# ixaxaar/lambda-cdm-raytracing

Measured on NVIDIA B200. Metric: pairwise_interactions_per_s, higher is better.
Workload: dtype f32

## Files before the change

lambda-cdm-raytracing_b200/csrc/capi.cu:

```cuda
#include <math.h>
#include <new>
#include <string.h>

#include "common.cuh"
#include "diag.cuh"
#include "direct.cuh"
#include "ics.cuh"
#include "leapfrog.cuh"
#include "pm.cuh"
#include "probe.cuh"
#include "shard.cuh"
#include "sort.cuh"
#include "tree.cuh"

using namespace b200;

static inline cudaStream_t pick_stream(b200_ctx*, void* stream) { return (cudaStream_t)stream; }

extern "C" {

const char* b200_error_string(int status) {
    switch (status) {
        case B200_OK: return "ok";
        case B200_ERR_INVALID: return "invalid argument";
        case B200_ERR_NO_DEVICE: return "no usable sm_100 CUDA device (there is no CPU fallback)";
        case B200_ERR_STATE: return "call out of order";
        case B200_ERR_NOMEM: return "device allocation failed";
        case B200_ERR_UNSUPPORTED: return "unsupported configuration";
        default: break;
    }
    if (status >= 1000 && status < 2000) return cudaGetErrorString((cudaError_t)(status - 1000));
    if (status >= 2000 && status < 3000) return shard_error_string(status - 2000);
    if (status >= 3000 && status < 4000) return "cuFFT error (status - 3000 is the cufftResult)";
    return "unknown b200grav status";
}

int b200_abi_version(void) { return B200GRAV_ABI_VERSION; }

int b200_ctx_create(int device, size_t max_particles, b200_ctx** out) {
    if (!out) return B200_ERR_INVALID;
    *out = nullptr;
    int count = 0;
    if (cudaGetDeviceCount(&count) != cudaSuccess || count == 0) {
        cudaGetLastError();
        return B200_ERR_NO_DEVICE;
    }
    if (device < 0 || device >= count) return B200_ERR_INVALID;
    cudaDeviceProp prop;
    B200_CUDA(cudaGetDeviceProperties(&prop, device));
    if (prop.major != 10) return B200_ERR_NO_DEVICE;
    B200_CUDA(cudaSetDevice(device));
    b200_ctx* ctx = new (std::nothrow) b200_ctx();
    if (!ctx) return B200_ERR_NOMEM;
    ctx->device = device;
    ctx->sm_count = prop.multiProcessorCount;
    cudaError_t ce = cudaStreamCreateWithFlags(&ctx->stream, cudaStreamNonBlocking);
    if (ce == cudaSuccess) ce = cudaEventCreate(&ctx->ev0);
    if (ce == cudaSuccess) ce = cudaEventCreate(&ctx->ev1);
    if (ce != cudaSuccess) { b200_ctx_destroy(ctx); return 1000 + (int)ce; }
    if (max_particles) {
        int s = ctx->src_tiles.reserve(direct_tiles_bytes(max_particles));
        if (s != B200_OK) { b200_ctx_destroy(ctx); return s; }
    }
    *out = ctx;
    return B200_OK;
}

int b200_ctx_destroy(b200_ctx* ctx) {
    if (!ctx) return B200_OK;
    cudaSetDevice(ctx->device);
    if (ctx->stream) cudaStreamSynchronize(ctx->stream);
    tree_destroy(ctx);
    shard_finalize(ctx);
    pm_destroy(ctx);
    ctx->src_tiles.release(); ctx->partials.release(); ctx->mass_flag.release(); ctx->zero_flag.release();
    ctx->energy_part.release(); ctx->energy_phi.release(); ctx->energy_out.release();
    ctx->ic_wk.release(); ctx->ic_tmp.release(); ctx->ic_psi.release(); ctx->ic_stats.release();
    ctx->h_pos3.release(); ctx->h_vel3.release(); ctx->h_mass.release(); ctx->h_posm4.release(); ctx->h_acc3.release();
    ctx->h_tree_posm4.release();
    ctx->probe.release(); ctx->sort_scratch.release();
    if (ctx->ev0) cudaEventDestroy(ctx->ev0);
    if (ctx->ev1) cudaEventDestroy(ctx->ev1);
    if (ctx->stream) cudaStreamDestroy(ctx->stream);
    delete ctx;
    return B200_OK;
}

int b200_ctx_device(const b200_ctx* ctx) { return ctx ? ctx->device : -1; }
int b200_ctx_sm_count(const b200_ctx* ctx) { return ctx ? ctx->sm_count : 0; }

void* b200_ctx_stream(const b200_ctx* ctx) { return ctx ? (void*)ctx->stream : nullptr; }

int b200_ctx_sync(b200_ctx* ctx, void* stream) {
    if (!ctx) return B200_ERR_INVALID;
    B200_CUDA(cudaStreamSynchronize(stream ? (cudaStream_t)stream : ctx->stream));
    return B200_OK;
}

int b200_direct_forces_dev(b200_ctx* ctx, const void* posm4, size_t n_sources, size_t i0,
                           size_t n_targets, float eps, float box, void* acc3, void* stream) {
    if (!ctx) return B200_ERR_INVALID;
    if (n_targets == 0) return B200_OK;
    if (!posm4 || !acc3 || i0 + n_targets > n_sources) return B200_ERR_INVALID;
    if (!(eps > 0.f) || box < 0.f) return B200_ERR_INVALID;
    B200_CUDA(cudaSetDevice(ctx->device));
    cudaStream_t st = pick_stream(ctx, stream);
    B200_TRY(ctx->src_tiles.reserve(direct_tiles_bytes(n_sources)));
    B200_TRY(ctx->mass_flag.reserve(sizeof(int)));
    B200_TRY(direct_pack_tiles(ctx, posm4, n_sources, ctx->src_tiles.as<float>(), ctx->mass_flag.as<int>(), st));
    DirectSources src;
    memset(&src, 0, sizeof src);
    src.n_parts = 1;
    src.tiles[0] = ctx->src_tiles.as<float>();
    src.total_tiles = src.tile_end[0] = (int)((n_sources + DIRECT_TILE_J - 1) / DIRECT_TILE_J);
    return direct_forces(ctx, src, (const float4*)posm4 + i0, n_targets, eps, box, acc3,
                         ctx->mass_flag.as<int>(), st);
}

int b200_direct_potential_dev(b200_ctx* ctx, const void* posm4, size_t n_sources, size_t i0,
                              size_t n_targets, float eps, float box, void* phi, void* stream) {
    if (!ctx) return B200_ERR_INVALID;
    if (n_targets == 0) return B200_OK;
    if (!posm4 || !phi || i0 + n_targets > n_sources) return B200_ERR_INVALID;
    if (!(eps > 0.f) || box < 0.f) return B200_ERR_INVALID;
    B200_CUDA(cudaSetDevice(ctx->device));
    cudaStream_t st = pick_stream(ctx, stream);
    B200_TRY(ctx->src_tiles.reserve(direct_tiles_bytes(n_sources)));
    B200_TRY(ctx->mass_flag.reserve(sizeof(int)));
    B200_TRY(direct_pack_tiles(ctx, posm4, n_sources, ctx->src_tiles.as<float>(), ctx->mass_flag.as<int>(), st));
    DirectSources src;
    memset(&src, 0, sizeof src);
    src.n_parts = 1;
    src.tiles[0] = ctx->src_tiles.as<float>();
    src.total_tiles = src.tile_end[0] = (int)((n_sources + DIRECT_TILE_J - 1) / DIRECT_TILE_J);
    return direct_potential(ctx, src, (const float4*)posm4 + i0, n_targets, eps, box, phi,
                            ctx->mass_flag.as<int>(), st);
}

int b200_energy_dev(b200_ctx* ctx, const void* posm4, size_t n_sources, size_t i0, size_t n_targets,
                    const void* vel3, float eps, float box, double* kinetic, double* potential,
                    void* stream) {
    if (!ctx || !kinetic || !potential) return B200_ERR_INVALID;
    *kinetic = *potential = 0.0;
    if (n_targets == 0) return B200_OK;
    if (!posm4 || !vel3 || i0 + n_targets > n_sources) return B200_ERR_INVALID;
    B200_CUDA(cudaSetDevice(ctx->device));
    cudaStream_t st = pick_stream(ctx, stream);
    B200_TRY(ctx->energy_phi.reserve(n_targets * sizeof(float)));
    B200_TRY(ctx->energy_out.reserve(2 * sizeof(double)));
    B200_TRY(b200_direct_potential_dev(ctx, posm4, n_sources, i0, n_targets, eps, box, ctx->energy_phi.p, stream));
    B200_TRY(energy_reduce(ctx, (const float4*)posm4 + i0, vel3, ctx->energy_phi.p, n_targets,
                           ctx->energy_out.as<double>(), st));
    double h[2];
    B200_CUDA(cudaMemcpyAsync(h, ctx->energy_out.p, sizeof h, cudaMemcpyDeviceToHost, st));
    B200_CUDA(cudaStreamSynchronize(st));
    *kinetic = h[0];
    *potential = h[1];
    return B200_OK;
}

int b200_force_error_dev(b200_ctx* ctx, const void* acc_test, const void* acc_ref, size_t n,
                         double* avg_rel_error, double* max_rel_error, void* stream) {
    if (!ctx || !avg_rel_error || !max_rel_error) return B200_ERR_INVALID;
    *avg_rel_error = *max_rel_error = 0.0;
    if (n == 0) return B200_OK;
    if (!acc_test || !acc_ref) return B200_ERR_INVALID;
    B200_CUDA(cudaSetDevice(ctx->device));
    return force_error(ctx, acc_test, acc_ref, n, avg_rel_error, max_rel_error, pick_stream(ctx, stream));
}
// ... 572 lines not shown
```

lambda-cdm-raytracing_b200/csrc/common.cuh:

```cuda
#pragma once
#ifdef B200_BOUNDS_CHECK
#include <assert.h>
#define B200_DEV_ASSERT(c) assert(c)
#else
#define B200_DEV_ASSERT(c) ((void)0)
#endif

#include <cuda_runtime.h>
#include <stddef.h>
#include <stdint.h>

#include "b200grav.h"

#define B200_CUDA(call)                                   \
    do {                                                  \
        cudaError_t e__ = (call);                         \
        if (e__ != cudaSuccess) return 1000 + (int)e__;   \
    } while (0)

#define B200_TRY(call)                  \
    do {                                \
        int s__ = (call);               \
        if (s__ != B200_OK) return s__; \
    } while (0)

struct DevBuf {
    void* p = nullptr;
    size_t bytes = 0;
    int reserve(size_t need) {
        if (need <= bytes) return B200_OK;
        if (p) cudaFree(p);
        p = nullptr; bytes = 0;
        size_t want = need + need / 8 + 256;
        cudaError_t e = cudaMalloc(&p, want);
        if (e != cudaSuccess) { cudaGetLastError(); return B200_ERR_NOMEM; }
        bytes = want;
        return B200_OK;
    }
    void release() { if (p) cudaFree(p); p = nullptr; bytes = 0; }
    template <class T> T* as() const { return (T*)p; }
};

namespace b200 { struct TreeState; struct ShardState; struct PmState; }

constexpr int B200_MAX_KERNEL_CFG = 64;
struct KernelCfg { const void* fn; int blocks_per_sm; };

struct b200_ctx {
    int device = 0;
    int sm_count = 0;
    cudaStream_t stream = nullptr;
    cudaEvent_t ev0 = nullptr, ev1 = nullptr;
    bool timing = false;
    float last_ms = 0.f;
    uint64_t launches = 0;
    KernelCfg kernel_cfg[B200_MAX_KERNEL_CFG];
    int n_kernel_cfg = 0;

    DevBuf src_tiles;
    DevBuf partials;
    DevBuf zero_flag;
    DevBuf mass_flag;
    DevBuf energy_part, energy_phi, energy_out;
    DevBuf ic_wk, ic_tmp, ic_psi, ic_stats;
    DevBuf h_pos3, h_vel3, h_mass, h_posm4, h_acc3;
    DevBuf h_tree_posm4;
    DevBuf probe, sort_scratch;

    b200::TreeState* tree = nullptr;
    b200::ShardState* shard = nullptr;
    b200::PmState* pm = nullptr;
};

static inline int ceil_div_i(long long a, long long b) { return (int)((a + b - 1) / b); }
```

lambda-cdm-raytracing_b200/csrc/direct.cu:

```cuda
#include <stdio.h>
#include <stdlib.h>

#include "common.cuh"
#include "direct.cuh"

namespace b200 {

namespace {

typedef unsigned long long u64;

__device__ __forceinline__ u64 pk(float lo, float hi) {
    u64 r;
    asm("mov.b64 %0, {%1, %2};" : "=l"(r) : "f"(lo), "f"(hi));
    return r;
}
__device__ __forceinline__ void unpk(u64 v, float& lo, float& hi) {
    asm("mov.b64 {%0, %1}, %2;" : "=f"(lo), "=f"(hi) : "l"(v));
}
__device__ __forceinline__ u64 add2(u64 a, u64 b) {
    u64 r;
    asm("add.rn.f32x2 %0, %1, %2;" : "=l"(r) : "l"(a), "l"(b));
    return r;
}
__device__ __forceinline__ u64 mul2(u64 a, u64 b) {
    u64 r;
    asm("mul.rn.f32x2 %0, %1, %2;" : "=l"(r) : "l"(a), "l"(b));
    return r;
}
__device__ __forceinline__ u64 fma2(u64 a, u64 b, u64 c) {
    u64 r;
    asm("fma.rn.f32x2 %0, %1, %2, %3;" : "=l"(r) : "l"(a), "l"(b), "l"(c));
    return r;
}
__device__ __forceinline__ float rsqrt_approx(float x) {
    float r;
    asm("rsqrt.approx.ftz.f32 %0, %1;" : "=f"(r) : "f"(x));
    return r;
}

__device__ __forceinline__ uint32_t smem_u32(const void* p) {
    return (uint32_t)__cvta_generic_to_shared(p);
}
__device__ __forceinline__ void mbar_init(uint64_t* bar, uint32_t count) {
    asm volatile("mbarrier.init.shared::cta.b64 [%0], %1;" ::"r"(smem_u32(bar)), "r"(count));
}
__device__ __forceinline__ void mbar_expect_tx(uint64_t* bar, uint32_t bytes) {
    asm volatile("mbarrier.arrive.expect_tx.shared::cta.b64 _, [%0], %1;" ::"r"(smem_u32(bar)),
                 "r"(bytes)
                 : "memory");
}
__device__ __forceinline__ void mbar_wait(uint64_t* bar, uint32_t parity) {
    asm volatile(
        "{\n"
        ".reg .pred p;\n"
        "WAIT_LOOP:\n"
        "mbarrier.try_wait.parity.shared::cta.b64 p, [%0], %1;\n"
        "@p bra WAIT_DONE;\n"
        "bra WAIT_LOOP;\n"
        "WAIT_DONE:\n"
        "}\n" ::"r"(smem_u32(bar)),
        "r"(parity)
        : "memory");
}
__device__ __forceinline__ void tma_load_1d(void* dst_smem, const void* src_gmem, uint32_t bytes,
                                            uint64_t* bar) {
    asm volatile(
        "cp.async.bulk.shared::cluster.global.mbarrier::complete_tx::bytes [%0], [%1], %2, [%3];" ::"r"(
            smem_u32(dst_smem)),
        "l"(src_gmem), "r"(bytes), "r"(smem_u32(bar))
        : "memory");
}

constexpr float FAR_AWAY = 1.0e18f;

__global__ void pack_tiles_kernel(const float4* __restrict__ posm, long long n, long long n_padded,
                                  float* __restrict__ tiles, int* __restrict__ mass_diff) {
    long long j = (long long)blockIdx.x * blockDim.x + threadIdx.x;
    if (j >= n_padded) return;
    float4 p = make_float4(FAR_AWAY, FAR_AWAY, FAR_AWAY, 0.f);
    if (j < n) {
        p = posm[j];
        if (mass_diff && p.w != posm[0].w) atomicAdd(mass_diff, 1);
    }
    long long t = j / DIRECT_TILE_J;
    int o = (int)(j % DIRECT_TILE_J);
    float* base = tiles + t * (4 * DIRECT_TILE_J) + o;
    base[0 * DIRECT_TILE_J] = p.x;
    base[1 * DIRECT_TILE_J] = p.y;
    base[2 * DIRECT_TILE_J] = p.z;
    base[3 * DIRECT_TILE_J] = p.w;
}

constexpr int STAGES = 4;
constexpr int TILE_J = DIRECT_TILE_J;
constexpr int TILE_FLOATS = 4 * TILE_J;
constexpr uint32_t TILE_BYTES = TILE_FLOATS * sizeof(float);

__device__ __forceinline__ const float* tile_ptr(const DirectSources& src, int t) {
    int p = 0, base = 0;
#pragma unroll 1
    while (p < src.n_parts - 1 && t >= src.tile_end[p]) { base = src.tile_end[p]; ++p; }
    return src.tiles[p] + (size_t)(t - base) * TILE_FLOATS;
}

constexpr int PMODE_OPEN = 0, PMODE_FLOAT = 1, PMODE_FIXED_XY = 2;

__device__ __forceinline__ uint32_t fixed_point(float x, double units_per_length) {
    uint32_t e = (uint32_t)(unsigned long long)__double2ll_rn((double)x * units_per_length);
    return e - (e >> 31);
}

__device__ __forceinline__ int sub3(uint32_t a, uint32_t b, uint32_t c) {
    int d;
    asm("vsub.s32.s32.s32.add %0, %1, %2, %3;" : "=r"(d) : "r"(a), "r"(b), "r"(c));
    return d;
}

template <int R, int THREADS, int MINB, int PMODE, bool UNIT, bool POT = false>
__global__ void __launch_bounds__(THREADS, MINB)
direct_kernel(const DirectSources src, const float4* __restrict__ targets, long long n_targets,
              float eps2, float box, double* __restrict__ partials, long long n_units, int n_tiles,
              const int* __restrict__ mass_diff) {
    constexpr bool PERIODIC = (PMODE == PMODE_FLOAT);
    constexpr bool FIXED = (PMODE == PMODE_FIXED_XY);
    static_assert(!(FIXED && POT), "the potential keeps the FP32 minimum image");
    if (mass_diff != nullptr) {
        const bool uniform = (*mass_diff == 0);
        if (uniform != UNIT) return;
    } else if (UNIT) {
        return;
    }
    constexpr int BLOCK_I = THREADS * R;
    extern __shared__ __align__(128) unsigned char smem_raw[];
    float* stage_buf = reinterpret_cast<float*>(smem_raw);
    uint64_t* full = reinterpret_cast<uint64_t*>(smem_raw + STAGES * TILE_BYTES);
    double* dsum = reinterpret_cast<double*>(smem_raw + STAGES * TILE_BYTES + 64);

    const int tid = threadIdx.x;
    const long long G = gridDim.x, c = blockIdx.x;
    const long long u0 = (c * n_units) / G, u1 = ((c + 1) * n_units) / G;
    if (u0 >= u1) return;
    const long long my_units = u1 - u0;

    if (tid == 0) {
#pragma unroll
        for (int s = 0; s < STAGES; ++s) mbar_init(&full[s], 1);
        asm volatile("fence.mbarrier_init.release.cluster;" ::: "memory");
    }
    __syncthreads();

    long long b = u0 / n_tiles;
    int t = (int)(u0 % n_tiles);

    if (tid == 0) {
        int tt = t;
        for (int k = 0; k < STAGES - 1 && k < my_units; ++k) {
            mbar_expect_tx(&full[k], TILE_BYTES);
            tma_load_1d(stage_buf + k * TILE_FLOATS, tile_ptr(src, tt), TILE_BYTES, &full[k]);
            if (++tt == n_tiles) tt = 0;
        }
    }
    int t_issue = (int)((u0 + (STAGES - 1)) % n_tiles);

    [[maybe_unused]] const double units = FIXED ? 4294967296.0 / (double)box : 1.0;
    [[maybe_unused]] const uint32_t zero = (uint32_t)(n_tiles >> 31);
    const u64 eps2_2 = pk(eps2, eps2);
    constexpr int RF = FIXED ? 1 : R, RI = FIXED ? R : 1;
    [[maybe_unused]] u64 nxi[RF], nyi[RF];
    u64 nzi[R];
    [[maybe_unused]] uint32_t ixi[RI], iyi[RI];
    auto load_targets = [&](long long blk) {
#pragma unroll
        for (int r = 0; r < R; ++r) {
            long long i = blk * BLOCK_I + r * THREADS + tid;
            float4 p = make_float4(0.f, 0.f, 0.f, 0.f);
            if (i < n_targets) p = targets[i];
            if constexpr (FIXED) {
                if (!(p.x == p.x) || !(p.y == p.y)) p.z = p.x + p.y;
                ixi[r] = fixed_point(p.x, units);
                iyi[r] = fixed_point(p.y, units);
            } else {
                nxi[r] = pk(-p.x, -p.x);
                nyi[r] = pk(-p.y, -p.y);
            }
// ... 91 lines not shown
                if constexpr (UNIT) f = mul2(f, rinv);
                else f = mul2(f, mul2(M, rinv));
                ax[r] = fma2(f, dx, ax[r]);
                ay[r] = fma2(f, dy, ay[r]);
                az[r] = fma2(f, dz, az[r]);
            }
        };

#pragma unroll 1
        for (int j4 = 0; j4 < TILE_J / 4; ++j4) {
            const ulonglong2 X = sx[j4], Y = sy[j4], Z = sz[j4];
            ulonglong2 M = make_ulonglong2(0ull, 0ull);
            if constexpr (!UNIT || FIXED) M = sm[j4];
            interact(X.x, Y.x, Z.x, M.x);
            interact(X.y, Y.y, Z.y, M.y);
        }

#pragma unroll
        for (int r = 0; r < R; ++r) {
            float lo, hi;
            unpk(ax[r], lo, hi); dsum[(0 * R + r) * THREADS + tid] += (double)(lo + hi);
            if constexpr (!POT) {
                unpk(ay[r], lo, hi); dsum[(1 * R + r) * THREADS + tid] += (double)(lo + hi);
                unpk(az[r], lo, hi); dsum[(2 * R + r) * THREADS + tid] += (double)(lo + hi);
            }
        }
        if constexpr (FIXED) asm volatile("fence.proxy.async.shared::cta;" ::: "memory");
        __syncthreads();

        ++t;
        const bool last = (k == my_units - 1);
        if (t == n_tiles || last) {
            double* rec = partials + (size_t)(c + b) * 3 * BLOCK_I;
#pragma unroll
            for (int r = 0; r < R; ++r) {
                rec[0 * BLOCK_I + r * THREADS + tid] = dsum[(0 * R + r) * THREADS + tid];
                if constexpr (!POT) {
                    rec[1 * BLOCK_I + r * THREADS + tid] = dsum[(1 * R + r) * THREADS + tid];
                    rec[2 * BLOCK_I + r * THREADS + tid] = dsum[(2 * R + r) * THREADS + tid];
                }
            }
            if (t == n_tiles) {
                t = 0;
                ++b;
                if (!last) load_targets(b);
            }
        }
    }
}

__global__ void direct_finalize_kernel(const double* __restrict__ partials, float* __restrict__ acc3,
                                       long long n_targets, int block_i, long long n_units,
                                       int n_tiles, int G, const int* __restrict__ mass_diff,
                                       const float* __restrict__ first_tile, double scale_xy) {
    long long i = (long long)blockIdx.x * blockDim.x + threadIdx.x;
    if (i >= n_targets) return;
    long long b = i / block_i;
    int o = (int)(i % block_i);
    long long uf = b * n_tiles, ul = uf + n_tiles - 1;
    long long cf = ((uf + 1) * G - 1) / n_units;
    long long cl = ((ul + 1) * G - 1) / n_units;
    double sx = 0.0, sy = 0.0, sz = 0.0;
    for (long long c = cf; c <= cl; ++c) {
        const double* rec = partials + (size_t)(c + b) * 3 * block_i;
        sx += rec[o];
        sy += rec[block_i + o];
        sz += rec[2 * block_i + o];
    }
    if (mass_diff != nullptr && *mass_diff == 0) {
        const double m0 = (double)first_tile[3 * DIRECT_TILE_J];
        sx *= m0; sy *= m0; sz *= m0;
    }
    acc3[3 * i + 0] = (float)(sx * scale_xy);
    acc3[3 * i + 1] = (float)(sy * scale_xy);
    acc3[3 * i + 2] = (float)sz;
}

__global__ void potential_finalize_kernel(const double* __restrict__ partials, const float4* __restrict__ targets,
                                          float* __restrict__ phi, long long n_targets, int block_i,
                                          long long n_units, int n_tiles, int G, float eps2,
                                          const int* __restrict__ mass_diff,
                                          const float* __restrict__ first_tile) {
    long long i = (long long)blockIdx.x * blockDim.x + threadIdx.x;
    if (i >= n_targets) return;
    long long b = i / block_i;
    int o = (int)(i % block_i);
    long long uf = b * n_tiles, ul = uf + n_tiles - 1;
    long long cf = ((uf + 1) * G - 1) / n_units;
    long long cl = ((ul + 1) * G - 1) / n_units;
    double s = 0.0;
    for (long long c = cf; c <= cl; ++c) s += partials[(size_t)(c + b) * 3 * block_i + o];
    const double self = (double)rsqrt_approx(eps2);
    if (mass_diff != nullptr && *mass_diff == 0) s = (s - self) * (double)first_tile[3 * DIRECT_TILE_J];
    else s -= self * (double)targets[i].w;
    phi[i] = (float)s;
}

constexpr int ENERGY_BLOCKS = 296;
__global__ void __launch_bounds__(256)
energy_partial_kernel(const float4* __restrict__ targets, const float* __restrict__ vel3,
                      const float* __restrict__ phi, long long n, double* __restrict__ part ) {
    __shared__ double sk[256], sp[256];
    double ke = 0.0, pe = 0.0;
    for (long long i = (long long)blockIdx.x * blockDim.x + threadIdx.x; i < n; i += (long long)gridDim.x * blockDim.x) {
        const float4 p = targets[i];
        const double vx = vel3[3 * i], vy = vel3[3 * i + 1], vz = vel3[3 * i + 2];
        ke += 0.5 * (double)p.w * (vx * vx + vy * vy + vz * vz);
        pe -= 0.5 * (double)p.w * (double)phi[i];
    }
    sk[threadIdx.x] = ke; sp[threadIdx.x] = pe;
    __syncthreads();
    for (int s = 128; s > 0; s >>= 1) {
        if (threadIdx.x < s) { sk[threadIdx.x] += sk[threadIdx.x + s]; sp[threadIdx.x] += sp[threadIdx.x + s]; }
        __syncthreads();
    }
    if (threadIdx.x == 0) { part[blockIdx.x] = sk[0]; part[gridDim.x + blockIdx.x] = sp[0]; }
}
__global__ void energy_final_kernel(const double* __restrict__ part, int nblocks, double* __restrict__ out2) {
    if (threadIdx.x < 2) {
        double s = 0.0;
        for (int b = 0; b < nblocks; ++b) s += part[threadIdx.x * nblocks + b];
        out2[threadIdx.x] = s;
    }
}

template <int R, int THREADS, int MINB, int PMODE, bool POT = false>
int launch_direct(b200_ctx* ctx, const DirectSources& src, const float4* targets, size_t n_targets,
                  float eps, float box, float* acc3, const int* mass_diff, cudaStream_t st) {
    constexpr int BLOCK_I = THREADS * R;
    auto kern_g = direct_kernel<R, THREADS, MINB, PMODE, false, POT>;
    auto kern_u = direct_kernel<R, THREADS, MINB, PMODE, true, POT>;
    const size_t smem = STAGES * TILE_BYTES + 64 + (size_t)3 * R * THREADS * sizeof(double);
    int blocks_per_sm = 0;
    for (int k = 0; k < ctx->n_kernel_cfg; ++k)
        if (ctx->kernel_cfg[k].fn == (const void*)kern_g) blocks_per_sm = ctx->kernel_cfg[k].blocks_per_sm;
    if (blocks_per_sm == 0) {
        int bu = 0;
        B200_CUDA(cudaFuncSetAttribute(kern_g, cudaFuncAttributeMaxDynamicSharedMemorySize, (int)smem));
        B200_CUDA(cudaFuncSetAttribute(kern_u, cudaFuncAttributeMaxDynamicSharedMemorySize, (int)smem));
        B200_CUDA(cudaOccupancyMaxActiveBlocksPerMultiprocessor(&blocks_per_sm, kern_g, THREADS, smem));
        B200_CUDA(cudaOccupancyMaxActiveBlocksPerMultiprocessor(&bu, kern_u, THREADS, smem));
        if (bu < blocks_per_sm) blocks_per_sm = bu;
        if (blocks_per_sm < 1) return B200_ERR_UNSUPPORTED;
        if (ctx->n_kernel_cfg < B200_MAX_KERNEL_CFG) {
            ctx->kernel_cfg[ctx->n_kernel_cfg].fn = (const void*)kern_g;
            ctx->kernel_cfg[ctx->n_kernel_cfg].blocks_per_sm = blocks_per_sm;
            ++ctx->n_kernel_cfg;
        }
    }
    const long long T = ((long long)n_targets + BLOCK_I - 1) / BLOCK_I;
    const int NT = src.total_tiles;
    const long long U = T * NT;
    long long G = (long long)ctx->sm_count * blocks_per_sm;
    if (G > U) G = U;
    B200_TRY(ctx->partials.reserve((size_t)(G + T) * 3 * BLOCK_I * sizeof(double)));
    if (ctx->timing) B200_CUDA(cudaEventRecord(ctx->ev0, st));
    kern_g<<<(unsigned)G, THREADS, smem, st>>>(src, targets, (long long)n_targets, eps * eps, box,
                                               ctx->partials.as<double>(), U, NT, mass_diff);
    if (mass_diff)
        kern_u<<<(unsigned)G, THREADS, smem, st>>>(src, targets, (long long)n_targets, eps * eps, box,
                                                   ctx->partials.as<double>(), U, NT, mass_diff);
    if (ctx->timing) B200_CUDA(cudaEventRecord(ctx->ev1, st));
    B200_CUDA(cudaGetLastError());
    const int fb = 256;
    if constexpr (POT)
        potential_finalize_kernel<<<(unsigned)((n_targets + fb - 1) / fb), fb, 0, st>>>(
            ctx->partials.as<double>(), targets, acc3, (long long)n_targets, BLOCK_I, U, NT, (int)G, eps * eps,
            mass_diff, src.tiles[0]);
    else {
        const double sxy = PMODE == PMODE_FIXED_XY ? (double)box / 4294967296.0 : 1.0;
        direct_finalize_kernel<<<(unsigned)((n_targets + fb - 1) / fb), fb, 0, st>>>(
            ctx->partials.as<double>(), acc3, (long long)n_targets, BLOCK_I, U, NT, (int)G, mass_diff,
            src.tiles[0], sxy);
    }
    B200_CUDA(cudaGetLastError());
    ctx->launches += mass_diff ? 3 : 2;
    return B200_OK;
}

}

size_t direct_tiles_bytes(size_t n) {
    size_t nt = (n + DIRECT_TILE_J - 1) / DIRECT_TILE_J;
    return nt * 4 * DIRECT_TILE_J * sizeof(float);
}

int direct_pack_tiles(b200_ctx* ctx, const void* posm4, size_t n, float* tiles, int* mass_diff,
                      cudaStream_t st) {
    size_t nt = (n + DIRECT_TILE_J - 1) / DIRECT_TILE_J;
    long long n_padded = (long long)nt * DIRECT_TILE_J;
    if (n_padded == 0) return B200_OK;
    if (mass_diff) B200_CUDA(cudaMemsetAsync(mass_diff, 0, sizeof(int), st));
    pack_tiles_kernel<<<(unsigned)((n_padded + 255) / 256), 256, 0, st>>>(
        (const float4*)posm4, (long long)n, n_padded, tiles, mass_diff);
    B200_CUDA(cudaGetLastError());
    ctx->launches += 1;
    return B200_OK;
}

int direct_forces(b200_ctx* ctx, const DirectSources& src, const void* targets4, size_t n_targets,
                  float eps, float box, void* acc3, const int* mass_diff, cudaStream_t st) {
    if (!(eps > 0.f) || box < 0.f) return B200_ERR_INVALID;
    if (n_targets == 0) return B200_OK;
    if (src.total_tiles <= 0) {
        B200_CUDA(cudaMemsetAsync(acc3, 0, n_targets * 3 * sizeof(float), st));
        return B200_OK;
    }
    const float4* tg = (const float4*)targets4;
    float* out = (float*)acc3;
    const long long units8 = (((long long)n_targets + 2047) / 2048) * (long long)src.total_tiles;
    const bool small = n_targets < 4 * 2048 || units8 < 4ll * ctx->sm_count;
    if (const char* v = getenv("B200_DIRECT_VARIANT")) {
        int r = 0, th = 0, mb = 0;
        if (sscanf(v, "%d,%d,%d", &r, &th, &mb) == 3 && box > 0.f) {
            const bool fp = getenv("B200_DIRECT_PERIODIC_FLOAT") != nullptr;
#define B200_PVARIANT(RR, TH, MB) \
    if (r == RR && th == TH && mb == MB) \
        return fp ? launch_direct<RR, TH, MB, PMODE_FLOAT>(ctx, src, tg, n_targets, eps, box, out, mass_diff, st) \
                  : launch_direct<RR, TH, MB, PMODE_FIXED_XY>(ctx, src, tg, n_targets, eps, box, out, mass_diff, st);
            B200_PVARIANT(4, 256, 1) B200_PVARIANT(8, 256, 1) B200_PVARIANT(4, 512, 1)
#undef B200_PVARIANT
            return B200_ERR_UNSUPPORTED;
        }
        if (sscanf(v, "%d,%d,%d", &r, &th, &mb) == 3 && box == 0.f) {
#define B200_VARIANT(RR, TH, MB) \
    if (r == RR && th == TH && mb == MB) \
        return launch_direct<RR, TH, MB, PMODE_OPEN>(ctx, src, tg, n_targets, eps, box, out, mass_diff, st);
            B200_VARIANT(2, 256, 2) B200_VARIANT(4, 256, 1) B200_VARIANT(4, 256, 2) B200_VARIANT(5, 256, 1)
            B200_VARIANT(6, 256, 1) B200_VARIANT(8, 256, 1) B200_VARIANT(4, 384, 1) B200_VARIANT(4, 512, 1)
            B200_VARIANT(3, 512, 1) B200_VARIANT(6, 128, 2) B200_VARIANT(8, 128, 2) B200_VARIANT(7, 256, 1)
            B200_VARIANT(6, 384, 1) B200_VARIANT(5, 384, 1) B200_VARIANT(8, 192, 1) B200_VARIANT(6, 320, 1)
            B200_VARIANT(10, 256, 1) B200_VARIANT(5, 128, 3) B200_VARIANT(4, 128, 4)
            B200_VARIANT(2, 256, 3) B200_VARIANT(2, 256, 4) B200_VARIANT(3, 256, 2) B200_VARIANT(3, 256, 3)
            B200_VARIANT(2, 512, 2) B200_VARIANT(2, 1024, 1) B200_VARIANT(1, 256, 8) B200_VARIANT(1, 512, 4)
#undef B200_VARIANT
            return B200_ERR_UNSUPPORTED;
        }
    }
    if (box > 0.f) {
        const long long units4 = (((long long)n_targets + 2047) / 2048) * (long long)src.total_tiles;
        const bool fixed_ok = eps >= 1e-4f * box && n_targets >= 4 * 2048 && units4 >= 4ll * ctx->sm_count &&
                              getenv("B200_DIRECT_PERIODIC_FLOAT") == nullptr;
        if (fixed_ok)
            return launch_direct<4, 512, 1, PMODE_FIXED_XY>(ctx, src, tg, n_targets, eps, box, out, mass_diff, st);
        return small ? launch_direct<2, 256, 2, PMODE_FLOAT>(ctx, src, tg, n_targets, eps, box, out, mass_diff, st)
                     : launch_direct<4, 256, 1, PMODE_FLOAT>(ctx, src, tg, n_targets, eps, box, out, mass_diff, st);
    }
    return small ? launch_direct<2, 256, 2, PMODE_OPEN>(ctx, src, tg, n_targets, eps, box, out, mass_diff, st)
                 : launch_direct<8, 256, 1, PMODE_OPEN>(ctx, src, tg, n_targets, eps, box, out, mass_diff, st);
}

int direct_potential(b200_ctx* ctx, const DirectSources& src, const void* targets4, size_t n_targets,
                     float eps, float box, void* phi, const int* mass_diff, cudaStream_t st) {
    if (!(eps > 0.f) || box < 0.f) return B200_ERR_INVALID;
    if (n_targets == 0) return B200_OK;
    if (src.total_tiles <= 0) {
        B200_CUDA(cudaMemsetAsync(phi, 0, n_targets * sizeof(float), st));
        return B200_OK;
    }
    const float4* tg = (const float4*)targets4;
    float* out = (float*)phi;
    const long long units6 = (((long long)n_targets + 1535) / 1536) * (long long)src.total_tiles;
    const bool small = n_targets < 4 * 1536 || units6 < 4ll * ctx->sm_count;
    if (box > 0.f) {
        return small ? launch_direct<2, 256, 2, PMODE_FLOAT, true>(ctx, src, tg, n_targets, eps, box, out, nullptr, st)
                     : launch_direct<4, 256, 1, PMODE_FLOAT, true>(ctx, src, tg, n_targets, eps, box, out, nullptr, st);
    }
    return small ? launch_direct<2, 256, 2, PMODE_OPEN, true>(ctx, src, tg, n_targets, eps, box, out, mass_diff, st)
                 : launch_direct<6, 256, 1, PMODE_OPEN, true>(ctx, src, tg, n_targets, eps, box, out, mass_diff, st);
}

int energy_reduce(b200_ctx* ctx, const void* targets4, const void* vel3, const void* phi, size_t n,
                  double* out2, cudaStream_t st) {
    B200_TRY(ctx->energy_part.reserve(2 * ENERGY_BLOCKS * sizeof(double)));
    energy_partial_kernel<<<ENERGY_BLOCKS, 256, 0, st>>>((const float4*)targets4, (const float*)vel3,
                                                         (const float*)phi, (long long)n,
                                                         ctx->energy_part.as<double>());
    energy_final_kernel<<<1, 32, 0, st>>>(ctx->energy_part.as<double>(), ENERGY_BLOCKS, out2);
    B200_CUDA(cudaGetLastError());
    ctx->launches += 2;
    return B200_OK;
}

}
```

lambda-cdm-raytracing_b200/csrc/direct.cuh:

```cuda
#pragma once
#include "common.cuh"

namespace b200 {

constexpr int DIRECT_TILE_J = 512;
constexpr int DIRECT_MAX_PARTS = 16;

struct DirectSources {
    const float* tiles[DIRECT_MAX_PARTS];
    int tile_end[DIRECT_MAX_PARTS];
    int n_parts;
    int total_tiles;
};

size_t direct_tiles_bytes(size_t n_particles);
int direct_pack_tiles(b200_ctx* ctx, const void* posm4, size_t n, float* tiles, int* mass_diff,
                      cudaStream_t st);
int direct_forces(b200_ctx* ctx, const DirectSources& src, const void* targets4, size_t n_targets,
                  float eps, float box, void* acc3, const int* mass_diff, cudaStream_t st);
int direct_potential(b200_ctx* ctx, const DirectSources& src, const void* targets4, size_t n_targets,
                     float eps, float box, void* phi, const int* mass_diff, cudaStream_t st);
int energy_reduce(b200_ctx* ctx, const void* targets4, const void* vel3, const void* phi, size_t n,
                  double* out2, cudaStream_t st);

}
```

Before: 2897 billion.

## Exploit Newton's third law with a symmetric mutual direct-force kernel

Adds a mutual (symmetric) direct-summation path for the open-boundary all-pairs case. Each pair is evaluated once and applied to both particles, with results accumulated as fixed-point 64-bit integers through atomics so the output stays deterministic. The tile packing pass now also collects coordinate and mass bounds, and a decide kernel uses them on the device to pick a fixed-point scale or fall back to the existing kernel. The aim is to roughly halve the pairwise arithmetic, at the cost of global atomics, extra memsets, and shared-memory reductions for the j-side forces.

Measured after the change: 4013 billion (median of 6 runs). 38.5% higher.

```diff
diff --git a/lambda-cdm-raytracing_b200/csrc/capi.cu b/lambda-cdm-raytracing_b200/csrc/capi.cu
--- a/lambda-cdm-raytracing_b200/csrc/capi.cu
+++ b/lambda-cdm-raytracing_b200/csrc/capi.cu
@@ -74,6 +74,7 @@
     shard_finalize(ctx);
     pm_destroy(ctx);
     ctx->src_tiles.release(); ctx->partials.release(); ctx->mass_flag.release(); ctx->zero_flag.release();
+    ctx->mutual_stats.release(); ctx->mutual_acc.release(); ctx->mutual_nan.release();
     ctx->energy_part.release(); ctx->energy_phi.release(); ctx->energy_out.release();
     ctx->ic_wk.release(); ctx->ic_tmp.release(); ctx->ic_psi.release(); ctx->ic_stats.release();
     ctx->h_pos3.release(); ctx->h_vel3.release(); ctx->h_mass.release(); ctx->h_posm4.release(); ctx->h_acc3.release();
@@ -107,14 +108,21 @@
     cudaStream_t st = pick_stream(ctx, stream);
     B200_TRY(ctx->src_tiles.reserve(direct_tiles_bytes(n_sources)));
     B200_TRY(ctx->mass_flag.reserve(sizeof(int)));
-    B200_TRY(direct_pack_tiles(ctx, posm4, n_sources, ctx->src_tiles.as<float>(), ctx->mass_flag.as<int>(), st));
+    const bool mutual = (i0 == 0 && n_targets == n_sources && (long long)n_sources >= MUTUAL_MIN_N);
+    DirectStats* stats = nullptr;
+    if (mutual) {
+        B200_TRY(ctx->mutual_stats.reserve(sizeof(DirectStats)));
+        stats = ctx->mutual_stats.as<DirectStats>();
+    }
+    B200_TRY(direct_pack_tiles(ctx, posm4, n_sources, ctx->src_tiles.as<float>(), ctx->mass_flag.as<int>(), st,
+                               stats));
     DirectSources src;
     memset(&src, 0, sizeof src);
     src.n_parts = 1;
     src.tiles[0] = ctx->src_tiles.as<float>();
     src.total_tiles = src.tile_end[0] = (int)((n_sources + DIRECT_TILE_J - 1) / DIRECT_TILE_J);
     return direct_forces(ctx, src, (const float4*)posm4 + i0, n_targets, eps, box, acc3,
-                         ctx->mass_flag.as<int>(), st);
+                         ctx->mass_flag.as<int>(), st, stats);
 }
 
 int b200_direct_potential_dev(b200_ctx* ctx, const void* posm4, size_t n_sources, size_t i0,
diff --git a/lambda-cdm-raytracing_b200/csrc/common.cuh b/lambda-cdm-raytracing_b200/csrc/common.cuh
--- a/lambda-cdm-raytracing_b200/csrc/common.cuh
+++ b/lambda-cdm-raytracing_b200/csrc/common.cuh
@@ -61,6 +61,9 @@
     DevBuf partials;
     DevBuf zero_flag;
     DevBuf mass_flag;
+    DevBuf mutual_stats;
+    DevBuf mutual_acc;
+    DevBuf mutual_nan;
     DevBuf energy_part, energy_phi, energy_out;
     DevBuf ic_wk, ic_tmp, ic_psi, ic_stats;
     DevBuf h_pos3, h_vel3, h_mass, h_posm4, h_acc3;
diff --git a/lambda-cdm-raytracing_b200/csrc/direct.cu b/lambda-cdm-raytracing_b200/csrc/direct.cu
--- a/lambda-cdm-raytracing_b200/csrc/direct.cu
+++ b/lambda-cdm-raytracing_b200/csrc/direct.cu
@@ -74,22 +74,50 @@
 
 constexpr float FAR_AWAY = 1.0e18f;
 
-__global__ void pack_tiles_kernel(const float4* __restrict__ posm, long long n, long long n_padded,
-                                  float* __restrict__ tiles, int* __restrict__ mass_diff) {
+__device__ __forceinline__ unsigned float_key(float f) {
+    const unsigned u = __float_as_uint(f);
+    return (u & 0x80000000u) ? ~u : (u | 0x80000000u);
+}
+__device__ __forceinline__ float key_float(unsigned k) {
+    return __uint_as_float((k & 0x80000000u) ? (k & 0x7fffffffu) : ~k);
+}
+
+__global__ void __launch_bounds__(256)
+pack_tiles_kernel(const float4* __restrict__ posm, long long n, long long n_padded,
+                  float* __restrict__ tiles, int* __restrict__ mass_diff, DirectStats* __restrict__ stats) {
     long long j = (long long)blockIdx.x * blockDim.x + threadIdx.x;
-    if (j >= n_padded) return;
     float4 p = make_float4(FAR_AWAY, FAR_AWAY, FAR_AWAY, 0.f);
     if (j < n) {
         p = posm[j];
         if (mass_diff && p.w != posm[0].w) atomicAdd(mass_diff, 1);
     }
-    long long t = j / DIRECT_TILE_J;
-    int o = (int)(j % DIRECT_TILE_J);
-    float* base = tiles + t * (4 * DIRECT_TILE_J) + o;
-    base[0 * DIRECT_TILE_J] = p.x;
-    base[1 * DIRECT_TILE_J] = p.y;
-    base[2 * DIRECT_TILE_J] = p.z;
-    base[3 * DIRECT_TILE_J] = p.w;
+    if (j < n_padded) {
+        long long t = j / DIRECT_TILE_J;
+        int o = (int)(j % DIRECT_TILE_J);
+        float* base = tiles + t * (4 * DIRECT_TILE_J) + o;
+        base[0 * DIRECT_TILE_J] = p.x;
+        base[1 * DIRECT_TILE_J] = p.y;
+        base[2 * DIRECT_TILE_J] = p.z;
+        base[3 * DIRECT_TILE_J] = p.w;
+    }
+    if (stats == nullptr) return;
+    __shared__ unsigned red[8][8];
+    const float v[4] = {p.x, p.y, p.z, fabsf(p.w)};
+    const int lane = threadIdx.x & 31, w = threadIdx.x >> 5;
+#pragma unroll
+    for (int c = 0; c < 4; ++c) {
+        const bool ok = j < n && isfinite(v[c]);
+        const unsigned k = float_key(v[c]);
+        const unsigned hi = __reduce_max_sync(0xffffffffu, ok ? k : 0u);
+        const unsigned lo = __reduce_max_sync(0xffffffffu, ok ? ~k : 0u);
+        if (lane == 0) { red[w][c] = hi; red[w][4 + c] = lo; }
+    }
+    __syncthreads();
+    if (threadIdx.x < 8) {
+        unsigned m = 0;
+        for (int k = 0; k < (int)(blockDim.x >> 5); ++k) m = max(m, red[k][threadIdx.x]);
+        if (m) atomicMax(&stats->key[threadIdx.x], m);
+    }
 }
 
 constexpr int STAGES = 4;
@@ -121,7 +149,7 @@
 __global__ void __launch_bounds__(THREADS, MINB)
 direct_kernel(const DirectSources src, const float4* __restrict__ targets, long long n_targets,
               float eps2, float box, double* __restrict__ partials, long long n_units, int n_tiles,
-              const int* __restrict__ mass_diff) {
+              const int* __restrict__ mass_diff, const MutualParams* __restrict__ mutual) {
     constexpr bool PERIODIC = (PMODE == PMODE_FLOAT);
     constexpr bool FIXED = (PMODE == PMODE_FIXED_XY);
     static_assert(!(FIXED && POT), "the potential keeps the FP32 minimum image");
@@ -131,6 +159,7 @@
     } else if (UNIT) {
         return;
     }
+    if (mutual != nullptr && mutual->use) return;
     constexpr int BLOCK_I = THREADS * R;
     extern __shared__ __align__(128) unsigned char smem_raw[];
     float* stage_buf = reinterpret_cast<float*>(smem_raw);
@@ -328,9 +357,10 @@
 __global__ void direct_finalize_kernel(const double* __restrict__ partials, float* __restrict__ acc3,
                                        long long n_targets, int block_i, long long n_units,
                                        int n_tiles, int G, const int* __restrict__ mass_diff,
-                                       const float* __restrict__ first_tile, double scale_xy) {
+                                       const float* __restrict__ first_tile, double scale_xy,
+                                       const MutualParams* __restrict__ mutual) {
     long long i = (long long)blockIdx.x * blockDim.x + threadIdx.x;
-    if (i >= n_targets) return;
+    if (i >= n_targets || (mutual != nullptr && mutual->use)) return;
     long long b = i / block_i;
     int o = (int)(i % block_i);
     long long uf = b * n_tiles, ul = uf + n_tiles - 1;
@@ -402,7 +432,8 @@
 
 template <int R, int THREADS, int MINB, int PMODE, bool POT = false>
 int launch_direct(b200_ctx* ctx, const DirectSources& src, const float4* targets, size_t n_targets,
-                  float eps, float box, float* acc3, const int* mass_diff, cudaStream_t st) {
+                  float eps, float box, float* acc3, const int* mass_diff, cudaStream_t st,
+                  const MutualParams* mutual = nullptr) {
     constexpr int BLOCK_I = THREADS * R;
     auto kern_g = direct_kernel<R, THREADS, MINB, PMODE, false, POT>;
     auto kern_u = direct_kernel<R, THREADS, MINB, PMODE, true, POT>;
@@ -432,10 +463,10 @@
     B200_TRY(ctx->partials.reserve((size_t)(G + T) * 3 * BLOCK_I * sizeof(double)));
     if (ctx->timing) B200_CUDA(cudaEventRecord(ctx->ev0, st));
     kern_g<<<(unsigned)G, THREADS, smem, st>>>(src, targets, (long long)n_targets, eps * eps, box,
-                                               ctx->partials.as<double>(), U, NT, mass_diff);
+                                               ctx->partials.as<double>(), U, NT, mass_diff, mutual);
     if (mass_diff)
         kern_u<<<(unsigned)G, THREADS, smem, st>>>(src, targets, (long long)n_targets, eps * eps, box,
-                                                   ctx->partials.as<double>(), U, NT, mass_diff);
+                                                   ctx->partials.as<double>(), U, NT, mass_diff, mutual);
     if (ctx->timing) B200_CUDA(cudaEventRecord(ctx->ev1, st));
     B200_CUDA(cudaGetLastError());
     const int fb = 256;
@@ -447,13 +478,336 @@
         const double sxy = PMODE == PMODE_FIXED_XY ? (double)box / 4294967296.0 : 1.0;
         direct_finalize_kernel<<<(unsigned)((n_targets + fb - 1) / fb), fb, 0, st>>>(
             ctx->partials.as<double>(), acc3, (long long)n_targets, BLOCK_I, U, NT, (int)G, mass_diff,
-            src.tiles[0], sxy);
+            src.tiles[0], sxy, mutual);
     }
     B200_CUDA(cudaGetLastError());
     ctx->launches += mass_diff ? 3 : 2;
     return B200_OK;
 }
 
+__global__ void mutual_decide_kernel(const DirectStats* __restrict__ stats, const int* __restrict__ mass_diff,
+                                     long long n, float eps2, MutualParams* __restrict__ out) {
+    const unsigned* k = stats->key;
+    double l2 = 0.0;
+    for (int c = 0; c < 3; ++c) {
+        const double d = (double)key_float(k[c]) - (double)key_float(~k[4 + c]);
+        l2 += d * d;
+    }
+    const bool unit = (*mass_diff == 0);
+    const double mmax = unit ? 1.0 : (double)key_float(k[3]);
+    const double mmin = unit ? 1.0 : (double)key_float(~k[7]);
+    const double bound = (double)n * mmax * 0.38490018 / (double)eps2 * (1.0 + 1.0 / 256);
+    int e = 0;
+    frexp(bound, &e);
+    const double q = ldexp(1.0, e - 62);
+    const double floor_sum = (double)n * mmin / (3.0 * l2);
+    MutualParams p;
+    p.use = (k[0] != 0u && isfinite(l2) && bound > 0.0 && isfinite(bound) && e - 62 > -120 && e - 62 < 100 &&
+             q <= ldexp(floor_sum, -30)) ? 1 : 0;
+    p.q = q;
+    p.inv_q = (float)ldexp(1.0, 62 - e);
+    *out = p;
+}
+
+__device__ __forceinline__ long long to_fixed(float v, float inv_q, bool& bad) {
+    bad |= !(fabsf(v) <= 3.0e38f);
+    return __float2ll_rn(v * inv_q);
+}
+
+template <int R, int THREADS, int MINB, bool UNIT>
+__global__ void __launch_bounds__(THREADS, MINB)
+direct_mutual_kernel(const float* __restrict__ tiles, long long n, int n_tiles, int n_rows, long long n_units,
+                     float eps2, const int* __restrict__ mass_diff, const MutualParams* __restrict__ mp,
+                     unsigned long long* __restrict__ acc , int* __restrict__ nan_flag ) {
+    if (!mp->use || (*mass_diff == 0) != UNIT) return;
+    constexpr int BLOCK_I = THREADS * R;
+    constexpr int TPB = BLOCK_I / TILE_J;
+    constexpr int WARPS = THREADS / 32;
+    static_assert(BLOCK_I % TILE_J == 0 && THREADS % 32 == 0 && TILE_J % 64 == 0, "tile geometry");
+    extern __shared__ __align__(128) unsigned char smem_raw[];
+    float* stage_buf = reinterpret_cast<float*>(smem_raw);
+    uint64_t* full = reinterpret_cast<uint64_t*>(smem_raw + STAGES * TILE_BYTES);
+    long long* isum = reinterpret_cast<long long*>(smem_raw + STAGES * TILE_BYTES + 64);
+    float* jw = reinterpret_cast<float*>(isum + 3 * R * THREADS);
+
+    const int tid = threadIdx.x, lane = tid & 31, warp = tid >> 5;
+    const long long G = gridDim.x, c = blockIdx.x;
+    const long long u0 = (c * n_units) / G, u1 = ((c + 1) * n_units) / G;
+    if (u0 >= u1) return;
+    const long long my_units = u1 - u0;
+    const float inv_q = mp->inv_q;
+
+    auto row_start = [&](long long I) { return I * n_tiles - (long long)TPB * I * (I - 1) / 2; };
+    long long lo = 0, hi = n_rows - 1;
+    while (lo < hi) {
+        const long long mid = (lo + hi + 1) / 2;
+        if (row_start(mid) <= u0) lo = mid; else hi = mid - 1;
+    }
+    long long I = lo;
+    int t = (int)(TPB * I + (u0 - row_start(I)));
+
+    if (tid == 0) {
+#pragma unroll
+        for (int s = 0; s < STAGES; ++s) mbar_init(&full[s], 1);
+        asm volatile("fence.mbarrier_init.release.cluster;" ::: "memory");
+    }
+    __syncthreads();
+    long long I_issue = I;
+    int t_issue = t;
+    auto advance = [&](long long& row, int& tile) { if (++tile == n_tiles) { ++row; tile = (int)(TPB * row); } };
+    if (tid == 0) {
+        for (int k = 0; k < STAGES - 1 && k < my_units; ++k) {
+            mbar_expect_tx(&full[k], TILE_BYTES);
+            tma_load_1d(stage_buf + k * TILE_FLOATS, tiles + (size_t)t_issue * TILE_FLOATS, TILE_BYTES, &full[k]);
+            advance(I_issue, t_issue);
+        }
+    }
+
+    const u64 eps2_2 = pk(eps2, eps2);
+    u64 nxi[R], nyi[R], nzi[R];
+    [[maybe_unused]] u64 mi[R];
+    unsigned ibad = 0;
+    auto load_targets = [&](long long blk) {
+#pragma unroll
+        for (int r = 0; r < R; ++r) {
+            const int o = r * THREADS + tid;
+            const long long tile = blk * TPB + o / TILE_J;
+            float x = FAR_AWAY, y = FAR_AWAY, z = FAR_AWAY, m = 0.f;
+            if (tile < n_tiles) {
+                const float* p = tiles + (size_t)tile * TILE_FLOATS + o % TILE_J;
+                x = p[0]; y = p[TILE_J]; z = p[2 * TILE_J]; m = p[3 * TILE_J];
+            }
+            nxi[r] = pk(-x, -x);
+            nyi[r] = pk(-y, -y);
+            nzi[r] = pk(-z, -z);
+            if constexpr (!UNIT) mi[r] = pk(m, m);
+            isum[(0 * R + r) * THREADS + tid] = 0;
+            isum[(1 * R + r) * THREADS + tid] = 0;
+            isum[(2 * R + r) * THREADS + tid] = 0;
+        }
+        ibad = 0;
+    };
+    load_targets(I);
+
+    for (long long k = 0; k < my_units; ++k) {
+        const int s = (int)(k % STAGES);
+        if (tid == 0 && k + (STAGES - 1) < my_units) {
+            const int sn = (int)((k + STAGES - 1) % STAGES);
+            mbar_expect_tx(&full[sn], TILE_BYTES);
+            tma_load_1d(stage_buf + sn * TILE_FLOATS, tiles + (size_t)t_issue * TILE_FLOATS, TILE_BYTES, &full[sn]);
+            advance(I_issue, t_issue);
+        }
+        mbar_wait(&full[s], (uint32_t)((k / STAGES) & 1));
+        const float* tile = stage_buf + s * TILE_FLOATS;
+        const bool mutual = t >= TPB * (I + 1);
+
+        u64 ax[R], ay[R], az[R];
+#pragma unroll
+        for (int r = 0; r < R; ++r) ax[r] = ay[r] = az[r] = 0ull;
+        auto fold_i = [&]() {
+#pragma unroll
+            for (int r = 0; r < R; ++r) {
+                bool bad = false;
+                float a, b;
+                unpk(ax[r], a, b); isum[(0 * R + r) * THREADS + tid] += to_fixed(a + b, inv_q, bad);
+                unpk(ay[r], a, b); isum[(1 * R + r) * THREADS + tid] += to_fixed(a + b, inv_q, bad);
+                unpk(az[r], a, b); isum[(2 * R + r) * THREADS + tid] += to_fixed(a + b, inv_q, bad);
+                ibad |= (unsigned)bad << r;
+                ax[r] = ay[r] = az[r] = 0ull;
+            }
+        };
+
+        if (!mutual) {
+            const ulonglong2* sx = reinterpret_cast<const ulonglong2*>(tile);
+            const ulonglong2* sy = sx + TILE_J / 4;
+            const ulonglong2* sz = sy + TILE_J / 4;
+            const ulonglong2* sm = sz + TILE_J / 4;
+            auto interact = [&](u64 X, u64 Y, u64 Z, u64 M) {
+#pragma unroll
+                for (int r = 0; r < R; ++r) {
+                    const u64 dx = add2(X, nxi[r]), dy = add2(Y, nyi[r]), dz = add2(Z, nzi[r]);
+                    u64 r2 = fma2(dx, dx, eps2_2);
+                    r2 = fma2(dy, dy, r2);
+                    r2 = fma2(dz, dz, r2);
+                    float r2a, r2b;
+                    unpk(r2, r2a, r2b);
+                    const u64 rinv = pk(rsqrt_approx(r2a), rsqrt_approx(r2b));
+                    u64 f = mul2(rinv, rinv);
+                    if constexpr (UNIT) f = mul2(f, rinv);
+                    else f = mul2(f, mul2(M, rinv));
+                    ax[r] = fma2(f, dx, ax[r]);
+                    ay[r] = fma2(f, dy, ay[r]);
+                    az[r] = fma2(f, dz, az[r]);
+                }
+            };
+#pragma unroll 1
+            for (int j4 = 0; j4 < TILE_J / 4; ++j4) {
+                const ulonglong2 X = sx[j4], Y = sy[j4], Z = sz[j4];
+                ulonglong2 M = make_ulonglong2(0ull, 0ull);
+                if constexpr (!UNIT) M = sm[j4];
+                interact(X.x, Y.x, Z.x, M.x);
+                interact(X.y, Y.y, Z.y, M.y);
+            }
+            fold_i();
+        } else {
+            const u64* sx = reinterpret_cast<const u64*>(tile);
+            const u64* sy = sx + TILE_J / 2;
+            const u64* sz = sy + TILE_J / 2;
+            const u64* sm = sz + TILE_J / 2;
+            float* jwarp = jw + warp * 3 * TILE_J;
+#pragma unroll 1
+            for (int g = 0; g < TILE_J / 64; ++g) {
+                u64 jx = 0ull, jy = 0ull, jz = 0ull;
+#pragma unroll 1
+                for (int st = 0; st < 32; ++st) {
+                    const int p = g * 32 + ((lane + st) & 31);
+                    const u64 X = sx[p], Y = sy[p], Z = sz[p];
+                    [[maybe_unused]] u64 M = 0ull;
+                    if constexpr (!UNIT) M = sm[p];
+                    u64 sx_ = 0ull, sy_ = 0ull, sz_ = 0ull;
+#pragma unroll
+                    for (int r = 0; r < R; ++r) {
+                        const u64 dx = add2(X, nxi[r]), dy = add2(Y, nyi[r]), dz = add2(Z, nzi[r]);
+                        u64 r2 = fma2(dx, dx, eps2_2);
+                        r2 = fma2(dy, dy, r2);
+                        r2 = fma2(dz, dz, r2);
+                        float r2a, r2b;
+                        unpk(r2, r2a, r2b);
+                        const u64 rinv = pk(rsqrt_approx(r2a), rsqrt_approx(r2b));
+                        const u64 f = mul2(mul2(rinv, rinv), rinv);
+                        u64 fi = f, fj = f;
+                        if constexpr (!UNIT) { fi = mul2(f, M); fj = mul2(f, mi[r]); }
+                        ax[r] = fma2(fi, dx, ax[r]);
+                        ay[r] = fma2(fi, dy, ay[r]);
+                        az[r] = fma2(fi, dz, az[r]);
+                        sx_ = fma2(fj, dx, sx_);
+                        sy_ = fma2(fj, dy, sy_);
+                        sz_ = fma2(fj, dz, sz_);
+                    }
+                    jx = add2(jx, sx_);
+                    jy = add2(jy, sy_);
+                    jz = add2(jz, sz_);
+                    const int from = (lane + 1) & 31;
+                    jx = __shfl_sync(0xffffffffu, jx, from);
+                    jy = __shfl_sync(0xffffffffu, jy, from);
+                    jz = __shfl_sync(0xffffffffu, jz, from);
+                }
+                u64* o = reinterpret_cast<u64*>(jwarp + g * 64) + lane;
+                o[0 * TILE_J / 2] = jx;
+                o[1 * TILE_J / 2] = jy;
+                o[2 * TILE_J / 2] = jz;
+                fold_i();
+            }
+        }
+        __syncthreads();
+
+        if (mutual) {
+            const long long jb = (long long)t * TILE_J;
+            for (int e = tid; e < 3 * TILE_J; e += THREADS) {
+                const int comp = e / TILE_J, jo = e % TILE_J;
+                const long long j = jb + jo;
+                bool bad = false;
+                long long sum = 0;
+#pragma unroll
+                for (int w = 0; w < WARPS; ++w) sum += to_fixed(jw[(w * 3 + comp) * TILE_J + jo], inv_q, bad);
+                if (j < n) {
+                    atomicAdd(acc + comp * n + j, (unsigned long long)(-sum));
+                    if (bad) atomicOr(nan_flag + j, 1);
+                }
+            }
+            __syncthreads();
+        }
+
+        advance(I, t);
+        if (t == TPB * I || k == my_units - 1) {
+            const long long row = (t == TPB * I) ? I - 1 : I;
+#pragma unroll
+            for (int r = 0; r < R; ++r) {
+                const long long i = row * BLOCK_I + r * THREADS + tid;
+                if (i < n) {
+                    atomicAdd(acc + 0 * n + i, (unsigned long long)isum[(0 * R + r) * THREADS + tid]);
+                    atomicAdd(acc + 1 * n + i, (unsigned long long)isum[(1 * R + r) * THREADS + tid]);
+                    atomicAdd(acc + 2 * n + i, (unsigned long long)isum[(2 * R + r) * THREADS + tid]);
+                    if ((ibad >> r) & 1u) atomicOr(nan_flag + i, 1);
+                }
+            }
+            if (t == TPB * I && k != my_units - 1) load_targets(I);
+        }
+    }
+}
+
+__global__ void mutual_finalize_kernel(const long long* __restrict__ acc, const int* __restrict__ nan_flag,
+                                       long long n, const MutualParams* __restrict__ mp,
+                                       const int* __restrict__ mass_diff, const float* __restrict__ first_tile,
+                                       float* __restrict__ acc3) {
+    const long long i = (long long)blockIdx.x * blockDim.x + threadIdx.x;
+    if (i >= n || !mp->use) return;
+    double scale = mp->q;
+    if (*mass_diff == 0) scale *= (double)first_tile[3 * DIRECT_TILE_J];
+    const bool bad = nan_flag[i] != 0;
+#pragma unroll
+    for (int c = 0; c < 3; ++c) acc3[3 * i + c] = bad ? __int_as_float(0x7fffffff) : (float)((double)acc[c * n + i] * scale);
+}
+
+template <int R, int THREADS, int MINB>
+int launch_mutual(b200_ctx* ctx, const DirectSources& src, const float4* targets, size_t n, float eps,
+                  float* acc3, const int* mass_diff, DirectStats* stats, cudaStream_t st) {
+    constexpr int BLOCK_I = THREADS * R;
+    constexpr int TPB = BLOCK_I / TILE_J;
+    constexpr int WARPS = THREADS / 32;
+    auto kern_g = direct_mutual_kernel<R, THREADS, MINB, false>;
+    auto kern_u = direct_mutual_kernel<R, THREADS, MINB, true>;
+    const size_t smem = STAGES * TILE_BYTES + 64 + (size_t)3 * R * THREADS * sizeof(long long) +
+                        (size_t)WARPS * 3 * TILE_J * sizeof(float);
+    int blocks_per_sm = 0;
+    for (int k = 0; k < ctx->n_kernel_cfg; ++k)
+        if (ctx->kernel_cfg[k].fn == (const void*)kern_g) blocks_per_sm = ctx->kernel_cfg[k].blocks_per_sm;
+    if (blocks_per_sm == 0) {
+        int bu = 0;
+        B200_CUDA(cudaFuncSetAttribute(kern_g, cudaFuncAttributeMaxDynamicSharedMemorySize, (int)smem));
+        B200_CUDA(cudaFuncSetAttribute(kern_u, cudaFuncAttributeMaxDynamicSharedMemorySize, (int)smem));
+        B200_CUDA(cudaOccupancyMaxActiveBlocksPerMultiprocessor(&blocks_per_sm, kern_g, THREADS, smem));
+        B200_CUDA(cudaOccupancyMaxActiveBlocksPerMultiprocessor(&bu, kern_u, THREADS, smem));
+        if (bu < blocks_per_sm) blocks_per_sm = bu;
+        if (blocks_per_sm < 1) return B200_ERR_UNSUPPORTED;
+        if (ctx->n_kernel_cfg < B200_MAX_KERNEL_CFG) {
+            ctx->kernel_cfg[ctx->n_kernel_cfg].fn = (const void*)kern_g;
+            ctx->kernel_cfg[ctx->n_kernel_cfg].blocks_per_sm = blocks_per_sm;
+            ++ctx->n_kernel_cfg;
+        }
+    }
+    const long long NT = src.total_tiles;
+    const long long T = ((long long)n + BLOCK_I - 1) / BLOCK_I;
+    const long long U = T * NT - (long long)TPB * T * (T - 1) / 2;
+    long long G = (long long)ctx->sm_count * blocks_per_sm;
+    if (G > U) G = U;
+    MutualParams* mp = &stats->params;
+    B200_TRY(ctx->mutual_acc.reserve(3 * n * sizeof(long long)));
+    B200_TRY(ctx->mutual_nan.reserve(n * sizeof(int)));
+    B200_CUDA(cudaMemsetAsync(ctx->mutual_acc.p, 0, 3 * n * sizeof(long long), st));
+    B200_CUDA(cudaMemsetAsync(ctx->mutual_nan.p, 0, n * sizeof(int), st));
+    mutual_decide_kernel<<<1, 1, 0, st>>>(stats, mass_diff, (long long)n, eps * eps, mp);
+    B200_CUDA(cudaGetLastError());
+    if (ctx->timing) B200_CUDA(cudaEventRecord(ctx->ev0, st));
+    const bool timing = ctx->timing;
+    ctx->timing = false;
+    int s = launch_direct<8, 256, 1, PMODE_OPEN>(ctx, src, targets, n, eps, 0.f, acc3, mass_diff, st, mp);
+    ctx->timing = timing;
+    B200_TRY(s);
+    kern_g<<<(unsigned)G, THREADS, smem, st>>>(src.tiles[0], (long long)n, (int)NT, (int)T, U, eps * eps, mass_diff,
+                                               mp, ctx->mutual_acc.as<unsigned long long>(), ctx->mutual_nan.as<int>());
+    kern_u<<<(unsigned)G, THREADS, smem, st>>>(src.tiles[0], (long long)n, (int)NT, (int)T, U, eps * eps, mass_diff,
+                                               mp, ctx->mutual_acc.as<unsigned long long>(), ctx->mutual_nan.as<int>());
+    if (ctx->timing) B200_CUDA(cudaEventRecord(ctx->ev1, st));
+    B200_CUDA(cudaGetLastError());
+    const int fb = 256;
+    mutual_finalize_kernel<<<(unsigned)((n + fb - 1) / fb), fb, 0, st>>>(
+        ctx->mutual_acc.as<long long>(), ctx->mutual_nan.as<int>(), (long long)n, mp, mass_diff, src.tiles[0], acc3);
+    B200_CUDA(cudaGetLastError());
+    ctx->launches += 4;
+    return B200_OK;
+}
+
 }
 
 size_t direct_tiles_bytes(size_t n) {
@@ -462,20 +816,22 @@
 }
 
 int direct_pack_tiles(b200_ctx* ctx, const void* posm4, size_t n, float* tiles, int* mass_diff,
-                      cudaStream_t st) {
+                      cudaStream_t st, DirectStats* stats) {
     size_t nt = (n + DIRECT_TILE_J - 1) / DIRECT_TILE_J;
     long long n_padded = (long long)nt * DIRECT_TILE_J;
     if (n_padded == 0) return B200_OK;
     if (mass_diff) B200_CUDA(cudaMemsetAsync(mass_diff, 0, sizeof(int), st));
+    if (stats) B200_CUDA(cudaMemsetAsync(stats, 0, sizeof(DirectStats), st));
     pack_tiles_kernel<<<(unsigned)((n_padded + 255) / 256), 256, 0, st>>>(
-        (const float4*)posm4, (long long)n, n_padded, tiles, mass_diff);
+        (const float4*)posm4, (long long)n, n_padded, tiles, mass_diff, stats);
     B200_CUDA(cudaGetLastError());
     ctx->launches += 1;
     return B200_OK;
 }
 
 int direct_forces(b200_ctx* ctx, const DirectSources& src, const void* targets4, size_t n_targets,
-                  float eps, float box, void* acc3, const int* mass_diff, cudaStream_t st) {
+                  float eps, float box, void* acc3, const int* mass_diff, cudaStream_t st,
+                  DirectStats* stats) {
     if (!(eps > 0.f) || box < 0.f) return B200_ERR_INVALID;
     if (n_targets == 0) return B200_OK;
     if (src.total_tiles <= 0) {
@@ -513,6 +869,8 @@
             return B200_ERR_UNSUPPORTED;
         }
     }
+    if (stats != nullptr && box == 0.f && src.n_parts == 1 && (long long)n_targets >= MUTUAL_MIN_N)
+        return launch_mutual<8, 256, 1>(ctx, src, tg, n_targets, eps, out, mass_diff, stats, st);
     if (box > 0.f) {
         const long long units4 = (((long long)n_targets + 2047) / 2048) * (long long)src.total_tiles;
         const bool fixed_ok = eps >= 1e-4f * box && n_targets >= 4 * 2048 && units4 >= 4ll * ctx->sm_count &&
diff --git a/lambda-cdm-raytracing_b200/csrc/direct.cuh b/lambda-cdm-raytracing_b200/csrc/direct.cuh
--- a/lambda-cdm-raytracing_b200/csrc/direct.cuh
+++ b/lambda-cdm-raytracing_b200/csrc/direct.cuh
@@ -13,11 +13,17 @@
     int total_tiles;
 };
 
+constexpr long long MUTUAL_MIN_N = 65536;
+
+struct MutualParams { int use; float inv_q; double q; };
+struct DirectStats { unsigned key[8]; MutualParams params; };
+
 size_t direct_tiles_bytes(size_t n_particles);
 int direct_pack_tiles(b200_ctx* ctx, const void* posm4, size_t n, float* tiles, int* mass_diff,
-                      cudaStream_t st);
+                      cudaStream_t st, DirectStats* stats = nullptr);
 int direct_forces(b200_ctx* ctx, const DirectSources& src, const void* targets4, size_t n_targets,
-                  float eps, float box, void* acc3, const int* mass_diff, cudaStream_t st);
+                  float eps, float box, void* acc3, const int* mass_diff, cudaStream_t st,
+                  DirectStats* stats = nullptr);
 int direct_potential(b200_ctx* ctx, const DirectSources& src, const void* targets4, size_t n_targets,
                      float eps, float box, void* phi, const int* mass_diff, cudaStream_t st);
 int energy_reduce(b200_ctx* ctx, const void* targets4, const void* vel3, const void* phi, size_t n,
```
